# marco-conciatori-public/weed_instance_segmentation

Measured on NVIDIA B200. Metric: msda_fwd_bwd_throughput, higher is better.
Workload: dtype bf16

## Files before the change

include/msda_b200.h:

```cpp
#ifndef MSDA_B200_H_
#define MSDA_B200_H_

#include <stddef.h>
#include <stdint.h>

#ifdef __cplusplus
extern "C" {
#endif

#define MSDA_B200_ABI_VERSION 12
#define MSDA_B200_MAX_LEVELS 8

#define MSDA_B200_F32 0
#define MSDA_B200_BF16 1
#define MSDA_B200_U8 2

#define MSDA_B200_OK 0
#define MSDA_B200_ERR_INVALID 1
#define MSDA_B200_ERR_UNSUPPORTED 2
#define MSDA_B200_ERR_CUDA 3
#define MSDA_B200_ERR_WORKSPACE 4

#define MSDA_B200_FLAG_PROFILE 1u
#define MSDA_B200_FLAG_BF16_ATOMICS 2u
#define MSDA_B200_FLAG_BWD_V1 4u
#define MSDA_B200_FLAG_BWD_V2 32u
#define MSDA_B200_FLAG_STRICT_PADDING 16u

typedef struct msda_b200_desc {
  int32_t B;
  int32_t S;
  int32_t Q;
  int32_t H;
  int32_t D;
  int32_t L;
  int32_t P;
  int32_t value_dtype;
  int32_t attn_dtype;
  uint32_t flags;
  const int32_t* spatial_shapes_hw;
  const int64_t* level_start_index;
} msda_b200_desc;

int msda_b200_abi_version(void);

const char* msda_b200_last_error(void);

int msda_b200_forward(const msda_b200_desc* desc, const void* value , const float* loc ,
                      const void* attn , void* out , const int32_t* query_order ,
                      void* stream);

size_t msda_b200_backward_workspace_bytes(const msda_b200_desc* desc);

int msda_b200_backward(const msda_b200_desc* desc, const void* value , const float* loc ,
                       const void* attn , const void* grad_out , void* grad_value ,
                       float* grad_loc , void* grad_attn , void* workspace ,
                       size_t workspace_bytes, const int32_t* query_order , void* stream);

int msda_b200_forward_fused(const msda_b200_desc* desc, const void* value , const void* offsets ,
                            const void* logits , const float* ref_points , void* out ,
                            float* attn_out , const int32_t* query_order , void* stream);

int msda_b200_backward_fused(const msda_b200_desc* desc, const void* value , const void* offsets ,
                             const void* logits , const float* ref_points , const void* grad_out ,
                             void* grad_value , void* grad_offsets , void* grad_logits ,
                             void* workspace , size_t workspace_bytes,
                             const int32_t* query_order , void* stream);

int msda_b200_add_layernorm_forward(const void* x , int x_dtype, const void* residual , int residual_dtype,
                                    const float* gamma , const float* beta , float eps, float* y ,
                                    void* y_lowp , float* mean , float* rstd ,
                                    int64_t rows, int32_t channels, void* stream);

int msda_b200_add_layernorm_backward(const float* grad_y , const void* grad_y_lowp ,
                                     const void* x , int x_dtype, const void* residual , int residual_dtype,
                                     const float* gamma , const float* mean , const float* rstd ,
                                     float* grad_sum , void* grad_sum_lowp , float* grad_gamma ,
                                     float* grad_beta , int64_t rows, int32_t channels, void* stream);

int msda_b200_add_layernorm_clamp_forward(const void* x , int x_dtype, const void* residual ,
                                          int residual_dtype, const float* gamma , const float* beta ,
                                          float eps, float clamp, float* y , void* y_lowp ,
                                          float* mean , float* rstd , int64_t rows,
                                          int32_t channels, void* stream);

int msda_b200_add_layernorm_clamp_backward(const float* grad_y , const void* grad_y_lowp ,
                                           const void* x , int x_dtype, const void* residual ,
                                           int residual_dtype, const float* gamma , const float* beta ,
                                           float clamp, const float* mean , const float* rstd ,
                                           float* grad_sum , void* grad_sum_lowp ,
                                           float* grad_gamma , float* grad_beta , int64_t rows,
                                           int32_t channels, void* stream);

// ... 73 lines not shown
```

weed_instance_segmentation_b200/_cabi.py:

```python
from __future__ import annotations

import ctypes
import os

PKG = os.path.dirname(os.path.abspath(__file__))
LIB_PATH = os.path.join(PKG, "libmsda_b200.so")

ABI_VERSION = 12
MAX_LEVELS = 8
F32, BF16, U8 = 0, 1, 2
FLAG_PROFILE = 1
FLAG_BF16_ATOMICS = 2
FLAG_BWD_V1 = 4
FLAG_STRICT_PADDING = 16
FLAG_BWD_V2 = 32
PROF_FWD, PROF_BWD_ZERO, PROF_BWD_MAIN, PROF_BWD_CONVERT = 0, 1, 2, 3

EXPORTS = (
    "msda_b200_abi_version",
    "msda_b200_last_error",
    "msda_b200_forward",
    "msda_b200_backward_workspace_bytes",
    "msda_b200_backward",
    "msda_b200_forward_fused",
    "msda_b200_backward_fused",
    "msda_b200_add_layernorm_forward",
    "msda_b200_add_layernorm_backward",
    "msda_b200_add_layernorm_clamp_forward",
    "msda_b200_add_layernorm_clamp_backward",
    "msda_b200_query_value_cast_forward",
    "msda_b200_query_value_cast_backward",
    "msda_b200_relu_backward_column_sum",
    "msda_b200_linear_f32_available",
    "msda_b200_linear_f32_forward",
    "msda_b200_linear_f32_grad_input",
    "msda_b200_linear_f32_grad_weight",
    "msda_b200_column_sum",
    "msda_b200_groupnorm_to_rows_forward",
    "msda_b200_groupnorm_to_rows_backward",
    "msda_b200_point_sample_forward",
    "msda_b200_point_sample_backward",
    "msda_b200_host_pipeline_create",
    "msda_b200_host_pipeline_step",
    "msda_b200_host_pipeline_join",
    "msda_b200_host_pipeline_sync",
    "msda_b200_host_pipeline_destroy",
    "msda_b200_profile_ms",
    "msda_b200_launch_count",
)


class Desc(ctypes.Structure):

    _fields_ = [
        ("B", ctypes.c_int32), ("S", ctypes.c_int32), ("Q", ctypes.c_int32), ("H", ctypes.c_int32),
        ("D", ctypes.c_int32), ("L", ctypes.c_int32), ("P", ctypes.c_int32),
        ("value_dtype", ctypes.c_int32), ("attn_dtype", ctypes.c_int32), ("flags", ctypes.c_uint32),
        ("spatial_shapes_hw", ctypes.POINTER(ctypes.c_int32)),
        ("level_start_index", ctypes.POINTER(ctypes.c_int64)),
    ]


class MSDAError(RuntimeError):

    def __init__(self, code: int, message: str):
        super().__init__(f"msda_b200 error {code}: {message}")
        self.code = code


_lib = None


def load() -> ctypes.CDLL:
    global _lib
    if _lib is not None:
        return _lib
    if not os.path.exists(LIB_PATH):
        raise ImportError(
            f"{LIB_PATH} is missing. Build it with `python -m weed_instance_segmentation_b200.build` "
            "(needs nvcc). This package has no CPU fallback."
        )
    lib = ctypes.CDLL(LIB_PATH)
    vp = ctypes.c_void_p
    dp = ctypes.POINTER(Desc)
    lib.msda_b200_abi_version.restype = ctypes.c_int
    lib.msda_b200_abi_version.argtypes = []
    lib.msda_b200_last_error.restype = ctypes.c_char_p
    lib.msda_b200_last_error.argtypes = []
    lib.msda_b200_forward.restype = ctypes.c_int
    lib.msda_b200_forward.argtypes = [dp, vp, vp, vp, vp, vp, vp]
    lib.msda_b200_backward_workspace_bytes.restype = ctypes.c_size_t
# ... 102 lines not shown
```

weed_instance_segmentation_b200/csrc/msda_b200.cu:

```cuda
#include <cuda_bf16.h>
#include <cuda_runtime.h>

#include <atomic>
#include <cstdarg>
#include <cstdio>
#include <cstring>
#include <type_traits>

#include "msda_b200.h"

namespace {

#include "msda_common.cuh"

template <int NT, int LPP, int QPG>
struct Tile {
  static constexpr int NG = NT / LPP;
  static constexpr int TQ = NG * QPG;
  static constexpr int ROW = TQ + 1;
};

__device__ __forceinline__ void decode_block(const KParams& p, int& b, int& tile, int& h) {
  int bid = blockIdx.x;
  h = bid % p.H;
  bid /= p.H;
  tile = bid % p.num_tiles;
  b = bid / p.num_tiles;
}

template <typename AT>
__device__ __forceinline__ float2 load_pair(const void* base, long long idx);
template <>
__device__ __forceinline__ float2 load_pair<float>(const void* base, long long idx) {
  return __ldg(reinterpret_cast<const float2*>(base) + idx);
}
template <>
__device__ __forceinline__ float2 load_pair<__nv_bfloat16>(const void* base, long long idx) {
  const __nv_bfloat162 v = reinterpret_cast<const __nv_bfloat162*>(base)[idx];
  return make_float2(__low2float(v), __high2float(v));
}
template <typename AT>
__device__ __forceinline__ void store_pair(void* base, long long idx, float x, float y);
template <>
__device__ __forceinline__ void store_pair<float>(void* base, long long idx, float x, float y) {
  reinterpret_cast<float2*>(base)[idx] = make_float2(x, y);
}
template <>
__device__ __forceinline__ void store_pair<__nv_bfloat16>(void* base, long long idx, float x, float y) {
  reinterpret_cast<__nv_bfloat162*>(base)[idx] = __floats2bfloat162_rn(x, y);
}

__device__ __forceinline__ float2 implicit_reference_point(const KParams& p, int q) {
  int lq = 0;
  for (int l = 1; l < p.L; ++l)
    if (q >= p.lv[l].start) lq = l;
  const int r = q - p.lv[lq].start, W = p.lv[lq].W, H = p.lv[lq].H;
  const int y = r / W, x = r - y * W;
  return make_float2(__fdiv_rn((float)x + 0.5f, (float)W), __fdiv_rn((float)y + 0.5f, (float)H));
}

template <typename AT>
__device__ __forceinline__ float2 fused_loc(const KParams& p, long long si, long long ri, int q, const Level& lv) {
  const float2 off = load_pair<AT>(p.offsets, si);
  const float2 r = p.ref ? __ldg(reinterpret_cast<const float2*>(p.ref) + ri) : implicit_reference_point(p, q);
  return make_float2(__fadd_rn(r.x, __fdiv_rn(off.x, (float)lv.W)), __fadd_rn(r.y, __fdiv_rn(off.y, (float)lv.H)));
}

template <typename AT>
__device__ __forceinline__ void softmax_stats(const AT* lg, int LP, float& mx, float& inv) {
  mx = -INFINITY;
  for (int s = 0; s < LP; ++s) mx = fmaxf(mx, to_float<AT>(lg[s]));
  float sum = 0.f;
  for (int s = 0; s < LP; ++s) sum += expf(to_float<AT>(lg[s]) - mx);
  inv = 1.f / sum;
}

template <typename AT>
__device__ __forceinline__ void softmax_stats_x4(const AT* lg, int LP, int sub, bool valid, float& mx, float& inv) {
  mx = -INFINITY;
  if (valid)
    for (int s = sub; s < LP; s += 4) mx = fmaxf(mx, to_float<AT>(lg[s]));
  mx = fmaxf(mx, __shfl_xor_sync(0xffffffffu, mx, 1));
  mx = fmaxf(mx, __shfl_xor_sync(0xffffffffu, mx, 2));
  float sum = 0.f;
  if (valid)
    for (int s = sub; s < LP; s += 4) sum += expf(to_float<AT>(lg[s]) - mx);
  sum += __shfl_xor_sync(0xffffffffu, sum, 1);
  sum += __shfl_xor_sync(0xffffffffu, sum, 2);
  inv = valid ? 1.f / sum : 0.f;
}

template <typename AT, int NT, int HPB>
__device__ __forceinline__ void tile_softmax(const KParams& p, int b, int h0, int q0, int nq, float* s_att, bool write_out) {
  const int LP = p.LP;
  const int sub = threadIdx.x & 3;
  const int nv = nq * HPB;
  for (int vb0 = 0; vb0 < nv; vb0 += NT / 4) {
    const int v = vb0 + (threadIdx.x >> 2);
    const bool valid = v < nv;
    const int ql = v / HPB, h = h0 + v % HPB;
    const int q = valid ? (p.q_order ? p.q_order[q0 + ql] : q0 + ql) : 0;
    const long long row = (((long long)b * p.Q + q) * p.H + h) * LP;
    const AT* lg = reinterpret_cast<const AT*>(p.logits) + row;
    if (LP <= 16) {
      float e[4];
      float mx = -INFINITY;
#pragma unroll
      for (int r = 0; r < 4; ++r) {
        const int s = sub + 4 * r;
        e[r] = (valid && s < LP) ? to_float<AT>(lg[s]) : -INFINITY;
// ... 564 lines not shown
    return fail(MSDA_B200_ERR_CUDA, "forward: cannot reserve %zu bytes of shared memory", smem);
  cudaFuncSetAttribute(kern, cudaFuncAttributePreferredSharedMemoryCarveout, FUSED ? -1 : 50);
  const long long blocks = (long long)p.B * p.num_tiles * (p.H / HPB);
  if (blocks > 0x7fffffffll) return fail(MSDA_B200_ERR_UNSUPPORTED, "forward: grid too large");
  {
    ProfScope ps((d->flags & MSDA_B200_FLAG_PROFILE) != 0, MSDA_B200_PROF_FWD, st);
    kern<<<(unsigned)blocks, NT, smem, st>>>(p);
    ++g_launches;
  }
  return check_launch("msda_b200_forward (head pairs)");
}

template <typename VT, typename AT, int D, int ACC, bool FUSED>
int launch_bwd(const msda_b200_desc* d, KParams p, cudaStream_t st) {
  constexpr int LPP = D / Vec16<VT>::N;
  using T = Tile<kBwdNT, LPP, kBwdQPG>;
  fill_geometry(d, p, T::TQ);
  const size_t n = (size_t)p.LP * T::ROW;
  const size_t smem = n * (2 * sizeof(float4) + sizeof(float) + sizeof(int)) +
                      (size_t)p.LP * T::TQ * LPP * sizeof(float4) +
                      (FUSED ? 2 * (size_t)T::TQ * p.LP * sizeof(float) : 0);
  auto kern = msda_bwd_kernel<VT, AT, D, kBwdNT, kBwdQPG, ACC, FUSED>;
  if (smem > 48 * 1024 &&
      cudaFuncSetAttribute(kern, cudaFuncAttributeMaxDynamicSharedMemorySize, (int)smem) != cudaSuccess)
    return fail(MSDA_B200_ERR_CUDA, "backward: cannot reserve %zu bytes of shared memory", smem);
  const long long blocks = (long long)p.B * p.num_tiles * p.H;
  if (blocks > 0x7fffffffll) return fail(MSDA_B200_ERR_UNSUPPORTED, "backward: grid too large");
  {
    ProfScope ps((d->flags & MSDA_B200_FLAG_PROFILE) != 0, MSDA_B200_PROF_BWD_MAIN, st);
    kern<<<(unsigned)blocks, kBwdNT, smem, st>>>(p);
    ++g_launches;
  }
  return check_launch("msda_b200_backward");
}

template <typename VT, typename AT, bool FUSED>
int dispatch_fwd(const msda_b200_desc* d, const KParams& p, cudaStream_t st) {
  if constexpr (std::is_same<VT, __nv_bfloat16>::value) {
    if (d->D == 32 && d->H % 2 == 0 && !(d->flags & MSDA_B200_FLAG_STRICT_PADDING))
      return launch_fwd_pair<VT, AT, 32, FUSED>(d, p, st);
  }
  switch (d->D) {
    case 8: return launch_fwd<VT, AT, 8, FUSED>(d, p, st);
    case 128: return launch_fwd<VT, AT, 128, FUSED>(d, p, st);
    case 16: return launch_fwd<VT, AT, 16, FUSED>(d, p, st);
    case 32: return launch_fwd<VT, AT, 32, FUSED>(d, p, st);
    case 64: return launch_fwd<VT, AT, 64, FUSED>(d, p, st);
  }
  return fail(MSDA_B200_ERR_UNSUPPORTED, "head dim %d", d->D);
}

constexpr int kSortNT = 256, kSortTQ = 128, kSortCAP = 2048;

bool sorted_applicable(const msda_b200_desc* d) {
  if (d->flags & MSDA_B200_FLAG_BWD_V1) return false;
  if (d->D != 32 || d->P != 4) return false;
  if (d->value_dtype != MSDA_B200_BF16) return false;
  for (int l = 0; l < d->L; ++l)
    if (d->spatial_shapes_hw[2 * l] > 4095 || d->spatial_shapes_hw[2 * l + 1] > 4095) return false;
  return true;
}

template <typename VT, typename AT, int ACC, bool FUSED, int kNT, int kTQ, int kPL>
int launch_bwd_sorted_cfg(const msda_b200_desc* d, KParams p, cudaStream_t st) {
  constexpr int D = 32, P = 4;
  constexpr int LPP = D / Vec16<VT>::N;
  fill_geometry(d, p, kTQ);
  const size_t smem = sorted_smem_layout<kNT, kTQ, P, kSortCAP, LPP>().total;
  auto kern = msda_bwd_sorted_kernel<VT, AT, D, kNT, kTQ, P, kSortCAP, ACC, FUSED, kPL>;
  if (cudaFuncSetAttribute(kern, cudaFuncAttributeMaxDynamicSharedMemorySize, (int)smem) != cudaSuccess)
    return fail(MSDA_B200_ERR_CUDA, "backward: cannot reserve %zu bytes of shared memory", smem);
  const long long blocks = (long long)p.B * p.num_tiles * p.H;
  if (blocks > 0x7fffffffll) return fail(MSDA_B200_ERR_UNSUPPORTED, "backward: grid too large");
  {
    ProfScope ps((d->flags & MSDA_B200_FLAG_PROFILE) != 0, MSDA_B200_PROF_BWD_MAIN, st);
    kern<<<(unsigned)blocks, kNT, smem, st>>>(p);
    ++g_launches;
  }
  return check_launch("msda_b200_backward (sorted)");
}

constexpr int kMmaNT = 256, kMmaTQ = 128, kMmaGCAP = 256, kMmaRCAP = 1024;

template <typename AT, bool FUSED>
int launch_bwd_mma(const msda_b200_desc* d, KParams p, cudaStream_t st) {
  constexpr int P = 4;
  fill_geometry(d, p, kMmaTQ);
  const size_t smem = mma_smem_layout<kMmaNT, kMmaTQ, P, kMmaGCAP, kMmaRCAP, FUSED>().total;
  auto kern = msda_bwd_mma_kernel<AT, kMmaNT, kMmaTQ, P, kMmaGCAP, kMmaRCAP, FUSED>;
  if (cudaFuncSetAttribute(kern, cudaFuncAttributeMaxDynamicSharedMemorySize, (int)smem) != cudaSuccess)
    return fail(MSDA_B200_ERR_CUDA, "backward: cannot reserve %zu bytes of shared memory", smem);
  const long long blocks = (long long)p.B * p.num_tiles * p.H;
  if (blocks > 0x7fffffffll) return fail(MSDA_B200_ERR_UNSUPPORTED, "backward: grid too large");
  {
    ProfScope ps((d->flags & MSDA_B200_FLAG_PROFILE) != 0, MSDA_B200_PROF_BWD_MAIN, st);
    kern<<<(unsigned)blocks, kMmaNT, smem, st>>>(p);
    ++g_launches;
  }
  return check_launch("msda_b200_backward (group-sorted, mma)");
}

template <typename VT, typename AT, int ACC, bool FUSED>
int dispatch_bwd(const msda_b200_desc* d, const KParams& p, cudaStream_t st) {
  if constexpr (std::is_same<VT, __nv_bfloat16>::value) {
    if (sorted_applicable(d)) {
      if constexpr (ACC == 0) {
        if (!(d->flags & MSDA_B200_FLAG_BWD_V2)) return launch_bwd_mma<AT, FUSED>(d, p, st);
      }
      return launch_bwd_sorted_cfg<VT, AT, ACC, FUSED, kSortNT, kSortTQ, 4>(d, p, st);
    }
  }
  switch (d->D) {
    case 8: return launch_bwd<VT, AT, 8, ACC, FUSED>(d, p, st);
    case 128: return launch_bwd<VT, AT, 128, ACC, FUSED>(d, p, st);
    case 16: return launch_bwd<VT, AT, 16, ACC, FUSED>(d, p, st);
    case 32: return launch_bwd<VT, AT, 32, ACC, FUSED>(d, p, st);
    case 64: return launch_bwd<VT, AT, 64, ACC, FUSED>(d, p, st);
  }
  return fail(MSDA_B200_ERR_UNSUPPORTED, "head dim %d", d->D);
}

template <bool FUSED>
int run_forward(const msda_b200_desc* desc, const KParams& p, cudaStream_t st) {
  const bool vbf = desc->value_dtype == MSDA_B200_BF16, abf = desc->attn_dtype == MSDA_B200_BF16;
  if (!vbf) return dispatch_fwd<float, float, FUSED>(desc, p, st);
  if (abf) return dispatch_fwd<__nv_bfloat16, __nv_bfloat16, FUSED>(desc, p, st);
  return dispatch_fwd<__nv_bfloat16, float, FUSED>(desc, p, st);
}

template <bool FUSED>
int run_backward(const msda_b200_desc* desc, KParams p, void* grad_value, void* workspace, size_t workspace_bytes,
                 bool have_tensors, cudaStream_t st) {
  const bool prof = (desc->flags & MSDA_B200_FLAG_PROFILE) != 0;
  const bool vbf = desc->value_dtype == MSDA_B200_BF16, abf = desc->attn_dtype == MSDA_B200_BF16;
  const bool bf16_atomics = vbf && (desc->flags & MSDA_B200_FLAG_BF16_ATOMICS);
  const size_t nvalue = (size_t)desc->B * desc->S * desc->H * desc->D;
  const size_t need = msda_b200_backward_workspace_bytes(desc);
  if (nvalue && !grad_value) return fail(MSDA_B200_ERR_INVALID, "backward: grad_value is NULL");
  if (need && nvalue && (!workspace || workspace_bytes < need))
    return fail(MSDA_B200_ERR_WORKSPACE, "backward: workspace of %zu bytes required, got %zu", need, workspace_bytes);
  if (nvalue && need && (reinterpret_cast<uintptr_t>(workspace) & 15))
    return fail(MSDA_B200_ERR_INVALID, "backward: workspace must be 16-byte aligned");

  void* acc = need ? workspace : grad_value;
  if (nvalue) {
    ProfScope ps(prof, MSDA_B200_PROF_BWD_ZERO, st);
    const size_t acc_bytes = need ? need : nvalue * dtype_size(desc->value_dtype);
    if (cudaMemsetAsync(acc, 0, acc_bytes, st) != cudaSuccess) return check_launch("backward: memset");
  }
  if ((long long)desc->B * desc->Q != 0) {
    if (!have_tensors) return fail(MSDA_B200_ERR_INVALID, "backward: NULL tensor pointer");
    p.grad_value_acc = acc;
    int rc;
    if (!vbf) rc = dispatch_bwd<float, float, 0, FUSED>(desc, p, st);
    else if (bf16_atomics) rc = abf ? dispatch_bwd<__nv_bfloat16, __nv_bfloat16, 1, FUSED>(desc, p, st)
                                    : dispatch_bwd<__nv_bfloat16, float, 1, FUSED>(desc, p, st);
    else rc = abf ? dispatch_bwd<__nv_bfloat16, __nv_bfloat16, 0, FUSED>(desc, p, st)
                  : dispatch_bwd<__nv_bfloat16, float, 0, FUSED>(desc, p, st);
    if (rc) return rc;
  }
  if (need && nvalue) {
    ProfScope ps(prof, MSDA_B200_PROF_BWD_CONVERT, st);
    const long long n8 = (long long)(nvalue / 8);
    const int blocks = (int)((n8 + 255) / 256 < 148 * 16 ? (n8 + 255) / 256 : 148 * 16);
    msda_cvt_f32_bf16_kernel<<<blocks, 256, 0, st>>>(reinterpret_cast<const float4*>(workspace),
                                                     reinterpret_cast<uint4*>(grad_value), n8);
    ++g_launches;
    if (int rc = check_launch("backward: convert")) return rc;
  }
  return MSDA_B200_OK;
}

}

extern "C" {

int msda_b200_internal_fail(int code, const char* msg) { return fail(code, "%s", msg); }
int msda_b200_internal_validate(const msda_b200_desc* desc) { return validate(desc); }
void msda_b200_internal_count_launch(void) { ++g_launches; }

int msda_b200_abi_version(void) { return MSDA_B200_ABI_VERSION; }

const char* msda_b200_last_error(void) { return g_err; }

int msda_b200_forward(const msda_b200_desc* desc, const void* value, const float* loc, const void* attn, void* out,
                      const int32_t* query_order, void* stream) {
  g_err[0] = 0;
  if (int rc = validate(desc)) return rc;
  if ((long long)desc->B * desc->Q == 0) return MSDA_B200_OK;
  if (!value || !loc || !attn || !out) return fail(MSDA_B200_ERR_INVALID, "forward: NULL tensor pointer");
  KParams p;
  memset(&p, 0, sizeof(p));
  p.value = value; p.loc = loc; p.attn = attn; p.out = out; p.q_order = query_order;
  return run_forward<false>(desc, p, reinterpret_cast<cudaStream_t>(stream));
}

int msda_b200_forward_fused(const msda_b200_desc* desc, const void* value, const void* offsets, const void* logits,
                            const float* ref_points, void* out, float* attn_out, const int32_t* query_order,
                            void* stream) {
  g_err[0] = 0;
  if (int rc = validate(desc)) return rc;
  if ((long long)desc->B * desc->Q == 0) return MSDA_B200_OK;
  if (!value || !offsets || !logits || !out) return fail(MSDA_B200_ERR_INVALID, "forward_fused: NULL tensor pointer");
  if (!ref_points && desc->Q != desc->S)
    return fail(MSDA_B200_ERR_INVALID, "forward_fused: implicit reference points (ref_points = NULL) need Q == S");
  KParams p;
  memset(&p, 0, sizeof(p));
  p.value = value; p.offsets = offsets; p.logits = logits; p.ref = ref_points; p.out = out; p.attn_out = attn_out;
  p.q_order = query_order;
  return run_forward<true>(desc, p, reinterpret_cast<cudaStream_t>(stream));
}

size_t msda_b200_backward_workspace_bytes(const msda_b200_desc* desc) {
  if (!desc) return 0;
  if (desc->value_dtype == MSDA_B200_BF16 && !(desc->flags & MSDA_B200_FLAG_BF16_ATOMICS))
    return (size_t)desc->B * desc->S * desc->H * desc->D * sizeof(float);
  return 0;
}

int msda_b200_backward(const msda_b200_desc* desc, const void* value, const float* loc, const void* attn,
                       const void* grad_out, void* grad_value, float* grad_loc, void* grad_attn, void* workspace,
                       size_t workspace_bytes, const int32_t* query_order, void* stream) {
  g_err[0] = 0;
  if (int rc = validate(desc)) return rc;
  KParams p;
  memset(&p, 0, sizeof(p));
  p.value = value; p.loc = loc; p.attn = attn; p.grad_out = grad_out;
  p.grad_loc = grad_loc; p.grad_attn = grad_attn; p.q_order = query_order;
  const bool have = value && loc && attn && grad_out && grad_loc && grad_attn;
  return run_backward<false>(desc, p, grad_value, workspace, workspace_bytes, have, reinterpret_cast<cudaStream_t>(stream));
}

int msda_b200_backward_fused(const msda_b200_desc* desc, const void* value, const void* offsets, const void* logits,
                             const float* ref_points, const void* grad_out, void* grad_value, void* grad_offsets,
                             void* grad_logits, void* workspace, size_t workspace_bytes, const int32_t* query_order,
                             void* stream) {
  g_err[0] = 0;
  if (int rc = validate(desc)) return rc;
  KParams p;
  memset(&p, 0, sizeof(p));
  p.value = value; p.offsets = offsets; p.logits = logits; p.ref = ref_points; p.grad_out = grad_out;
  p.grad_offsets = grad_offsets; p.grad_logits = grad_logits; p.q_order = query_order;
  if (!ref_points && desc->Q != desc->S)
    return fail(MSDA_B200_ERR_INVALID, "backward_fused: implicit reference points (ref_points = NULL) need Q == S");
  const bool have = value && offsets && logits && grad_out && grad_offsets && grad_logits;
  return run_backward<true>(desc, p, grad_value, workspace, workspace_bytes, have, reinterpret_cast<cudaStream_t>(stream));
}

int msda_b200_profile_ms(int which, float* ms) {
  if (which < 0 || which >= MSDA_B200_PROF_COUNT || !ms) return fail(MSDA_B200_ERR_INVALID, "profile_ms: bad argument");
  if (g_prof.device < 0 || !g_prof.valid[which]) return fail(MSDA_B200_ERR_INVALID, "profile_ms: nothing recorded");
  const cudaError_t e = cudaEventElapsedTime(ms, g_prof.ev[which][0], g_prof.ev[which][1]);
  if (e != cudaSuccess) return fail(MSDA_B200_ERR_CUDA, "profile_ms: %s", cudaGetErrorString(e));
  return MSDA_B200_OK;
}

int64_t msda_b200_launch_count(int reset) {
  return reset ? g_launches.exchange(0) : g_launches.load();
}

}
```

weed_instance_segmentation_b200/csrc/msda_bwd_mma.cuh:

```cuda

__device__ __forceinline__ void ldsm_x4(unsigned (&r)[4], unsigned addr) {
  asm("ldmatrix.sync.aligned.m8n8.x4.shared.b16 {%0, %1, %2, %3}, [%4];"
      : "=r"(r[0]), "=r"(r[1]), "=r"(r[2]), "=r"(r[3]) : "r"(addr));
}
__device__ __forceinline__ void ldsm_x4_trans(unsigned (&r)[4], unsigned addr) {
  asm("ldmatrix.sync.aligned.m8n8.x4.trans.shared.b16 {%0, %1, %2, %3}, [%4];"
      : "=r"(r[0]), "=r"(r[1]), "=r"(r[2]), "=r"(r[3]) : "r"(addr));
}
__device__ __forceinline__ void ldsm_x2_trans(unsigned (&r)[2], unsigned addr) {
  asm("ldmatrix.sync.aligned.m8n8.x2.trans.shared.b16 {%0, %1}, [%2];" : "=r"(r[0]), "=r"(r[1]) : "r"(addr));
}
__device__ __forceinline__ unsigned movm_trans(unsigned x) {
  unsigned y;
  asm("movmatrix.sync.aligned.m8n8.trans.b16 %0, %1;" : "=r"(y) : "r"(x));
  return y;
}
__device__ __forceinline__ void mma_bf16(float (&d)[4], unsigned a0, unsigned a1, unsigned a2, unsigned a3, unsigned b0,
                                         unsigned b1) {
  asm("mma.sync.aligned.m16n8k16.row.col.f32.bf16.bf16.f32 {%0, %1, %2, %3}, {%4, %5, %6, %7}, {%8, %9}, "
      "{%0, %1, %2, %3};"
      : "+f"(d[0]), "+f"(d[1]), "+f"(d[2]), "+f"(d[3]) : "r"(a0), "r"(a1), "r"(a2), "r"(a3), "r"(b0), "r"(b1));
}

__device__ __forceinline__ int go_swizzle(int row) { return ((row >> 1) & 1) | ((row >> 3) & 2); }

#ifndef MSDA_MMA_MOVM
#define MSDA_MMA_MOVM 1
#endif

struct MmaSmem {
  size_t w, go, wrow, dot, a, xy, cnt, item, id, fb, misc, stat, total;
};

constexpr int kMmaItemRows = 64;

template <int NT, int TQ, int P, int GCAP, int RCAP, bool FUSED>
__host__ __device__ inline MmaSmem mma_smem_layout() {
  constexpr int NS = TQ * P;
  MmaSmem s;
  size_t o = 0;
  s.w = o;    o += sizeof(float4) * NS;
  s.go = o;   o += 64 * (TQ + 1);
  s.wrow = o; o += 16 * RCAP;
  s.dot = o;  o += sizeof(float4) * NS;
  s.a = o;    o += sizeof(float) * NS;
  s.xy = o;   o += sizeof(int) * NS;
  s.cnt = o;  o += sizeof(int) * GCAP;
  s.item = o; o += sizeof(uint2) * (GCAP + RCAP / kMmaItemRows + 8);
  s.id = o;   o += sizeof(unsigned) * RCAP;
  s.fb = o;   o += sizeof(unsigned short) * NS * 4;
  o = (o + 15) & ~size_t(15);
  s.misc = o; o += sizeof(int) * 64;
  s.stat = o;
  s.total = o;
  return s;
}

enum { MI_NITEMS = 9 };

template <typename AT, int NT, int TQ, int P, int GCAP, int RCAP, bool FUSED>
__global__ void __launch_bounds__(NT, 4) msda_bwd_mma_kernel(const __grid_constant__ KParams p) {
  using VT = __nv_bfloat16;
  constexpr int LPP = 4;
  constexpr int G = NT / LPP;
  constexpr int NS = TQ * P;
  constexpr int LP2 = Log2P<P>::v;
  constexpr int NW = NT / 32;
  static_assert(GCAP == NT, "the scan gives every thread one group counter");
  static_assert(NS % NT == 0, "every thread owns NS/NT samples per level");
  static_assert(NS <= 512, "row code: 9 bits of sample index");
  static_assert(RCAP < 2048 && RCAP % 16 == 0, "row index is 11 bits in the item word");
  extern __shared__ __align__(16) unsigned char smem_raw[];
  const MmaSmem lay = mma_smem_layout<NT, TQ, P, GCAP, RCAP, FUSED>();
  float4* s_w = reinterpret_cast<float4*>(smem_raw + lay.w);
  unsigned* s_go32 = reinterpret_cast<unsigned*>(smem_raw + lay.go);
  uint4* s_wrow = reinterpret_cast<uint4*>(smem_raw + lay.wrow);
  float* s_dot = reinterpret_cast<float*>(smem_raw + lay.dot);
  float* s_a = reinterpret_cast<float*>(smem_raw + lay.a);
  int* s_xy = reinterpret_cast<int*>(smem_raw + lay.xy);
  int* s_cnt = reinterpret_cast<int*>(smem_raw + lay.cnt);
  uint2* s_item = reinterpret_cast<uint2*>(smem_raw + lay.item);
  unsigned* s_id = reinterpret_cast<unsigned*>(smem_raw + lay.id);
  unsigned short* s_fb = reinterpret_cast<unsigned short*>(smem_raw + lay.fb);
  int* const s_misc2 = reinterpret_cast<int*>(smem_raw + lay.misc);

  int b, tile, h;
  decode_block(p, b, tile, h);
  const int q0 = tile * TQ;
  const int nq = min(TQ, p.Q - q0);
  const int tid = threadIdx.x, lane = tid & 31, warp = tid >> 5;
  const int g = tid / LPP, c = tid % LPP;
  const unsigned gmask = ((1u << LPP) - 1u) << ((lane / LPP) * LPP);
  const long long acc_base = (long long)b * p.batch_stride16;
  const uint4* const vrow = reinterpret_cast<const uint4*>(p.value) + acc_base;
  float* const acc_f = reinterpret_cast<float*>(p.grad_value_acc) + acc_base * 8;
  const unsigned go_sa = (unsigned)__cvta_generic_to_shared(s_go32);
  const unsigned wrow_sa = (unsigned)__cvta_generic_to_shared(s_wrow);

  constexpr int SPT = NS / NT;
  float2 pre_loc[SPT];
  float pre_a[SPT];
  float2 f_ref[SPT];
#pragma unroll
  for (int r = 0; r < SPT; ++r) {
    f_ref[r] = make_float2(0.f, 0.f);
    const int ql = (r * NT + tid) >> LP2;
    if (FUSED && !p.ref && ql < nq) f_ref[r] = implicit_reference_point(p, p.q_order ? p.q_order[q0 + ql] : q0 + ql);
  }
  auto fetch_level = [&](int l) {
#pragma unroll
    for (int r = 0; r < SPT; ++r) {
      const int si = r * NT + tid;
      const int ql = si >> LP2, pt = si & (P - 1);
      pre_loc[r] = make_float2(0.f, 0.f);
      pre_a[r] = 0.f;
      if (l < p.L && ql < nq) {
        const int q = p.q_order ? p.q_order[q0 + ql] : q0 + ql;
        const long long gi = (((long long)b * p.Q + q) * p.H + h) * p.LP + l * P + pt;
        if (FUSED) {
          const float2 off = load_pair<AT>(p.offsets, gi);
          const float2 rp = p.ref ? __ldg(reinterpret_cast<const float2*>(p.ref) + ((long long)b * p.Q + q) * p.L + l)
                                  : f_ref[r];
          pre_loc[r] = make_float2(__fadd_rn(rp.x, __fdiv_rn(off.x, (float)p.lv[l].W)),
                                   __fadd_rn(rp.y, __fdiv_rn(off.y, (float)p.lv[l].H)));
          pre_a[r] = to_float<AT>(reinterpret_cast<const AT*>(p.logits)[gi]);
        } else {
          pre_loc[r] = __ldg(reinterpret_cast<const float2*>(p.loc) + gi);
          pre_a[r] = to_float<AT>(reinterpret_cast<const AT*>(p.attn)[gi]);
        }
      }
    }
  };
  fetch_level(0);

  for (int i = tid; i < TQ * LPP; i += NT) {
    const int ql = i >> 2, cc = i & 3;
    uint4 v = make_uint4(0u, 0u, 0u, 0u);
    if (ql < nq) {
      const int q = p.q_order ? p.q_order[q0 + ql] : q0 + ql;
      v = ldg16(reinterpret_cast<const uint4*>(p.grad_out) + (((long long)b * p.Q + q) * p.H + h) * LPP + cc);
    }
    const int sw = go_swizzle(ql);
    unsigned* row = s_go32 + ql * 16 + cc;
    row[(0 ^ sw) << 2] = __byte_perm(v.x, v.z, 0x5410);
    row[(1 ^ sw) << 2] = __byte_perm(v.x, v.z, 0x7632);
    row[(2 ^ sw) << 2] = __byte_perm(v.y, v.w, 0x5410);
    row[(3 ^ sw) << 2] = __byte_perm(v.y, v.w, 0x7632);
  }
  if (tid < 16) s_go32[TQ * 16 + tid] = 0u;

  static_assert(!FUSED || P == 4, "fused prologue: four lanes per (query, head) row");
  float f_lse[SPT], f_dsum[SPT];
#pragma unroll
  for (int r = 0; r < SPT; ++r) { f_lse[r] = 0.f; f_dsum[r] = 0.f; }
  if (FUSED) {
#pragma unroll
    for (int r = 0; r < SPT; ++r) {
      const int ql = (r * NT + tid) >> LP2;
      const bool valid = ql < nq;
      const int q = valid ? (p.q_order ? p.q_order[q0 + ql] : q0 + ql) : 0;
      float mx, inv;
      softmax_stats_x4<AT>(reinterpret_cast<const AT*>(p.logits) + (((long long)b * p.Q + q) * p.H + h) * p.LP, p.LP,
                           tid & 3, valid, mx, inv);
      f_lse[r] = valid ? mx - logf(inv) : 0.f;
    }
  }

  auto init_misc = [&](int* m) {
    int init = 0;
    if (tid == MI_MINX || tid == MI_MINY) init = 0x7fffffff;
// ... 96 lines not shown
              if (((cn & 1) ? cx1 : cx0) && ((cn & 2) ? cy1 : cy0))
                s_fb[atomicAdd(&s_misc[MI_FBN], 1)] = (unsigned short)(si * 4 + cn);
          }
        }
        code[r][k] = cd;
      }
    }
    __syncthreads();

    {
      const int cnt = s_cnt[tid];
      const int v = cnt | (((cnt + kMmaItemRows - 1) / kMmaItemRows) << 16);
      int incl = v;
#pragma unroll
      for (int off = 1; off < 32; off <<= 1) {
        const int t = __shfl_up_sync(0xffffffffu, incl, off);
        if (lane >= off) incl += t;
      }
      if (lane == 31) s_misc[MI_WSUM + warp] = incl;
      __syncthreads();
      int base = 0;
#pragma unroll
      for (int w2 = 0; w2 < NW; ++w2)
        if (w2 < warp) base += s_misc[MI_WSUM + w2];
      const int excl = base + incl - v;
      const int row_start = excl & 0xffff, item_start = excl >> 16;
      s_cnt[tid] = row_start;
      if (tid == NT - 1) {
        s_misc[MI_TOTAL] = (excl + v) & 0xffff;
        s_misc[MI_NITEMS] = (excl + v) >> 16;
      }
      if (cnt > 0) {
        const int gyl = tid / gw, gxl = tid - gyl * gw;
        const int px0 = (gx_lo + gxl) << 2, py0 = (gy_lo + gyl) << 1;
        const unsigned xbits = (1u << min(lv.W - px0, 4)) - 1u;
        const unsigned mask = xbits | (py0 + 1 < lv.H ? xbits << 4 : 0u);
        const unsigned pixoff = (unsigned)((py0 * lv.W + px0) * (p.H * LPP));
        for (int j = 0; j * kMmaItemRows < cnt; ++j) {
          const int rb = row_start + j * kMmaItemRows;
          const int n = rb < RCAP ? min(min(kMmaItemRows, cnt - j * kMmaItemRows), RCAP - rb) : 0;
          s_item[item_start + j] = make_uint2((unsigned)(n ? rb : 0) | ((unsigned)n << 11) | (mask << 18), pixoff);
        }
      }
    }
    __syncthreads();

#pragma unroll
    for (int r = 0; r < SPT; ++r) {
      const int si = r * NT + tid;
      const int xy = s_xy[si];
      const int x = xy & 0xfff, y = (xy >> 12) & 0xfff;
      const float4 w = s_w[si];
      const float a = s_a[si];
#pragma unroll
      for (int k = 0; k < 4; ++k) {
        const int cd = code[r][k];
        if (cd >= 0) {
          const int ci = k & 1, cj = k >> 1;
          const int slot = atomicAdd(&s_cnt[cd], 1);
          if (slot < RCAP) {
            const int bx = ci ? -1 : (x & 3), by = cj ? -1 : (y & 1);
            const int ql = si >> LP2;
            s_id[slot] = (unsigned)(ql * 64 + (go_swizzle(ql) << 4)) | ((unsigned)(si | ((bx + 1) << 9) | ((by + 1) << 12)) << 14);
            const float y0w = by == 0 ? a * w.z : (by == -1 ? a * w.w : 0.f);
            const float y1w = by == 1 ? a * w.z : (by == 0 ? a * w.w : 0.f);
            const unsigned p0 = Vec16<VT>::pack2(y0w * w.x, y0w * w.y), p1 = Vec16<VT>::pack2(y1w * w.x, y1w * w.y);
            const unsigned long long r0 = bx >= 0 ? ((unsigned long long)p0 << (16 * bx)) : (unsigned long long)(p0 >> 16);
            const unsigned long long r1 = bx >= 0 ? ((unsigned long long)p1 << (16 * bx)) : (unsigned long long)(p1 >> 16);
            s_wrow[slot] = make_uint4((unsigned)r0, (unsigned)(r0 >> 32), (unsigned)r1, (unsigned)(r1 >> 32));
          } else {
            const int gcode = xy >> 24;
            const bool ax0 = (gcode & 3) != 1, ax1 = ((gcode >> 2) & 3) != 1;
            const bool ay0 = ((gcode >> 4) & 3) != 1, ay1 = ((gcode >> 6) & 3) != 1;
            const bool xsplit = (x & 3) == 3, ysplit = (y & 1) == 1;
            const bool cx0 = (ci == 0) && ax0, cx1 = ax1 && (ci == 0 ? !xsplit : xsplit);
            const bool cy0 = (cj == 0) && ay0, cy1 = ay1 && (cj == 0 ? !ysplit : ysplit);
#pragma unroll
            for (int cn = 0; cn < 4; ++cn)
              if (((cn & 1) ? cx1 : cx0) && ((cn & 2) ? cy1 : cy0))
                s_fb[atomicAdd(&s_misc[MI_FBN], 1)] = (unsigned short)(si * 4 + cn);
          }
        }
      }
    }
    __syncthreads();
    s_cnt[tid] = 0;

    {
      const int g8 = lane >> 2, t4 = lane & 3;
      const int n_items = s_misc[MI_NITEMS];
      const int pix16 = p.H * LPP;
      const uint4* const v_lane = vrow + (lv.start * p.H + h) * LPP + ((g8 >> 2) * lv.W + (g8 & 3)) * pix16 + t4;
      float* const acc_lane = acc_f + (long long)((lv.start * p.H + h) * LPP + ((t4 >> 1) * lv.W + 2 * (t4 & 1)) * pix16) * 8 + 4 * g8;
      const int kx = 2 * (t4 & 1) + 1, ky = (t4 >> 1) + 1;
      const unsigned vbit = 1u << (18 + g8), fbit = 1u << (18 + 2 * t4);
      const unsigned lsel = ((unsigned)lane >> 4) << 4;
      auto load_v = [&](uint2 item) -> uint4 {
        if (item.x & vbit) return ldg16(v_lane + (int)item.y);
        return make_uint4(0u, 0u, 0u, 0u);
      };
      int it = warp;
      uint2 item = it < n_items ? s_item[it] : make_uint2(0u, 0u);
      uint4 vv = load_v(item);
      while (it < n_items) {
        const int it_n = it + NW;
        const uint2 item_n = it_n < n_items ? s_item[it_n] : make_uint2(0u, 0u);
        const uint4 vv_n = load_v(item_n);
        const int n = (int)((item.x >> 11) & 127u);
        if (n != 0) {
          const int rbeg = (int)(item.x & 0x7ffu), rend = rbeg + n;
          const unsigned bv00 = __byte_perm(vv.x, vv.z, 0x5410);
          const unsigned bv01 = __byte_perm(vv.x, vv.z, 0x7632);
          const unsigned bv10 = __byte_perm(vv.y, vv.w, 0x5410);
          const unsigned bv11 = __byte_perm(vv.y, vv.w, 0x7632);
          float acc0[4] = {0.f, 0.f, 0.f, 0.f}, acc1[4] = {0.f, 0.f, 0.f, 0.f};
          const unsigned kNoRow = 0x0fffc000u | (unsigned)(TQ * 64);
          int r0 = rbeg;
          unsigned code_l = r0 + (lane & 15) < rend ? s_id[r0 + (lane & 15)] : kNoRow;
          while (true) {
            const int rn = r0 + 16;
            const unsigned code_ln = rn + (lane & 15) < rend ? s_id[rn + (lane & 15)] : kNoRow;
            const int idx = r0 + (lane & 15);
            const unsigned ga = go_sa + ((code_l & 0x3fffu) ^ lsel);
            unsigned a[4], a2[4], tA[4], tB[4], bw[2];
            ldsm_x4(a, ga);
            ldsm_x4(a2, ga ^ 32u);
#if MSDA_MMA_MOVM
#pragma unroll
            for (int j = 0; j < 4; ++j) { tA[j] = movm_trans(a[j]); tB[j] = movm_trans(a2[j]); }
#else
            ldsm_x4_trans(tA, ga);
            ldsm_x4_trans(tB, ga ^ 32u);
#endif
            ldsm_x2_trans(bw, idx < rend ? wrow_sa + idx * 16 : go_sa + TQ * 64);
            float d[4] = {0.f, 0.f, 0.f, 0.f};
            mma_bf16(d, a[0], a[1], a[2], a[3], bv00, bv01);
            mma_bf16(d, a2[0], a2[1], a2[2], a2[3], bv10, bv11);
            mma_bf16(acc0, tA[0], tA[2], tA[1], tA[3], bw[0], bw[1]);
            mma_bf16(acc1, tB[0], tB[2], tB[1], tB[3], bw[0], bw[1]);
#pragma unroll
            for (int e = 0; e < 2; ++e) {
              const unsigned code = __shfl_sync(0xffffffffu, code_l, g8 + 8 * e);
              const int cxa = kx - (int)((code >> 23) & 7u), cy = ky - (int)((code >> 26) & 3u);
              float* dst = s_dot + ((code >> 14) & 511u) * 4 + cy * 2 + cxa;
              if ((unsigned)cy < 2u && (unsigned)cxa < 2u) dst[0] = d[2 * e];
              if ((unsigned)cy < 2u && (unsigned)(cxa + 1) < 2u) dst[1] = d[2 * e + 1];
            }
            if (rn >= rend) break;
            r0 = rn; code_l = code_ln;
          }
          float* const dst = acc_lane + (long long)(int)item.y * 8;
#pragma unroll
          for (int s = 0; s < 2; ++s) {
            const float v0 = acc0[s], v1 = acc0[2 + s], v2 = acc1[s], v3 = acc1[2 + s];
            const unsigned nz = (__float_as_uint(v0) | __float_as_uint(v1) | __float_as_uint(v2) | __float_as_uint(v3)) << 1;
            if ((item.x & (fbit << s)) && nz != 0u) red_add_f32x4(dst + s * pix16 * 8, v0, v1, v2, v3);
          }
        }
        it = it_n; item = item_n; vv = vv_n;
      }
    }

    fetch_level(l + 1);

    {
      const int nfb = s_misc[MI_FBN];
// ... 6 lines not shown
        const int x = (xy & 0xfff) + (cn & 1), y = ((xy >> 12) & 0xfff) + ((cn >> 1) & 1);
        const long long off = (long long)((lv.start + y * lv.W + x) * p.H + h) * LPP;
        float vf[8], gf[8];
        Vec16<VT>::unpack(ldg16(vrow + off + c), vf);
        {
          const int ql = si >> LP2, sw = go_swizzle(ql);
          const unsigned* row = s_go32 + ql * 16 + c;
#pragma unroll
          for (int j = 0; j < 4; ++j) {
            const unsigned u = row[(j ^ sw) << 2];
            gf[j] = __uint_as_float(u << 16);
            gf[j + 4] = __uint_as_float(u & 0xffff0000u);
          }
        }
        float d = 0.f;
#pragma unroll
        for (int j = 0; j < 8; ++j) d = fmaf(gf[j], vf[j], d);
#pragma unroll
        for (int o = 1; o < LPP; o <<= 1) d += __shfl_xor_sync(gmask, d, o);
        if (c == 0) s_dot[id] = d;
        if (wgt != 0.f) {
          float* dst = acc_f + (off + c) * 8;
          red_add_f32x4(dst, wgt * gf[0], wgt * gf[1], wgt * gf[2], wgt * gf[3]);
          red_add_f32x4(dst + 4, wgt * gf[4], wgt * gf[5], wgt * gf[6], wgt * gf[7]);
        }
      }
    }
    __syncthreads();

#pragma unroll
    for (int r = 0; r < SPT; ++r) {
      const int si = r * NT + tid;
      const int ql = si >> LP2, pt = si & (P - 1);
      const bool valid = ql < nq;
      const int q = valid ? (p.q_order ? p.q_order[q0 + ql] : q0 + ql) : 0;
      const long long gi = (((long long)b * p.Q + q) * p.H + h) * p.LP + l * P + pt;
      float4 d = *reinterpret_cast<const float4*>(&s_dot[si * 4]);
      const float4 w = s_w[si];
      const int gcode = s_xy[si] >> 24;
      const float a = s_a[si];
      const float gl = gdec(gcode, 0), gr = gdec(gcode, 1), gt = gdec(gcode, 2), gb = gdec(gcode, 3);
      d.x = (gl != 0.f && gt != 0.f) ? d.x : 0.f;
      d.y = (gr != 0.f && gt != 0.f) ? d.y : 0.f;
      d.z = (gl != 0.f && gb != 0.f) ? d.z : 0.f;
      d.w = (gr != 0.f && gb != 0.f) ? d.w : 0.f;
      const float top_s = w.x * d.x + w.y * d.y, bot_s = w.x * d.z + w.y * d.w;
      const float top_g = gl * d.x + gr * d.y, bot_g = gl * d.z + gr * d.w;
      const float g_attn = w.z * top_s + w.w * bot_s;
      const float g_px = w.z * top_g + w.w * bot_g, g_py = gt * top_s + gb * bot_s;
      if (!FUSED) {
        if (valid) {
          reinterpret_cast<AT*>(p.grad_attn)[gi] = from_float<AT>(g_attn);
          reinterpret_cast<float2*>(p.grad_loc)[gi] = make_float2((float)lv.W * a * g_px, (float)lv.H * a * g_py);
        }
      } else {
        if (valid) {
          store_pair<AT>(p.grad_offsets, gi, a * g_px, a * g_py);
          reinterpret_cast<AT*>(p.grad_logits)[gi] = from_float<AT>(g_attn);
        }
        float t = valid ? a * g_attn : 0.f;
#pragma unroll
        for (int o = 1; o < P; o <<= 1) t += __shfl_xor_sync(0xffffffffu, t, o);
        f_dsum[r] += t;
      }
    }
  }

  if (FUSED) {
#pragma unroll
    for (int r = 0; r < SPT; ++r) {
      const int ql = (r * NT + tid) >> LP2, pt = tid & (P - 1);
      if (ql < nq) {
        const int q = p.q_order ? p.q_order[q0 + ql] : q0 + ql;
        const long long row = (((long long)b * p.Q + q) * p.H + h) * p.LP;
        for (int l = 0; l < p.L; ++l) {
          const long long gi = row + l * P + pt;
          const float a = expf(to_float<AT>(reinterpret_cast<const AT*>(p.logits)[gi]) - f_lse[r]);
          const float ga = to_float<AT>(reinterpret_cast<const AT*>(p.grad_logits)[gi]);
          reinterpret_cast<AT*>(p.grad_logits)[gi] = from_float<AT>(a * (ga - f_dsum[r]));
        }
      }
    }
  }
}
```

weed_instance_segmentation_b200/csrc/msda_common.cuh:

```cuda
#pragma once

constexpr int kMaxL = MSDA_B200_MAX_LEVELS;

struct Level {
  int H, W;
  int start;
  int dx16;
  int dy16;
};

struct KParams {
  const void* value;
  const float* loc;
  const void* attn;
  void* out;
  const void* grad_out;
  void* grad_value_acc;
  float* grad_loc;
  void* grad_attn;
  const int* q_order;
  const void* offsets;
  const void* logits;
  const float* ref;
  float* attn_out;
  void* grad_offsets;
  void* grad_logits;
  int B, S, Q, H, L, P, LP;
  int num_tiles;
  long long batch_stride16;
  Level lv[kMaxL];
};

struct Axis {
  float s0, s1;
  float g0, g1;
  int base;
  bool ok;
};

__device__ __forceinline__ Axis axis_setup(float coord, int n) {
  Axis a;
  const float g = __fadd_rn(__fmul_rn(2.f, coord), -1.f);
  const float pix = __fmul_rn(__fadd_rn(__fmul_rn(__fadd_rn(g, 1.f), (float)n), -1.f), 0.5f);
  a.ok = (pix > -2.f) && (pix < (float)(n + 1));
  const float fl = floorf(pix);
  const int i0 = __float2int_rd(pix);
  const float l = pix - fl;
  const bool v0 = (i0 >= 0) && (i0 < n);
  const bool v1 = (i0 + 1 >= 0) && (i0 + 1 < n);
  const float w0 = v0 ? 1.f - l : 0.f, w1 = v1 ? l : 0.f;
  const float d0 = v0 ? -1.f : 0.f, d1 = v1 ? 1.f : 0.f;
  const int ib = min(max(i0, 0), max(n - 2, 0));
  const int shift = i0 - ib;
  a.base = ib;
  a.s0 = (shift == 0) ? w0 : ((shift == -1) ? w1 : 0.f);
  a.g0 = (shift == 0) ? d0 : ((shift == -1) ? d1 : 0.f);
  a.s1 = (shift == 0) ? w1 : ((shift == 1) ? w0 : 0.f);
  a.g1 = (shift == 0) ? d1 : ((shift == 1) ? d0 : 0.f);
  if (!a.ok) a.s0 = a.s1 = a.g0 = a.g1 = 0.f;
  return a;
}

template <typename T>
__device__ __forceinline__ float to_float(T v);
template <>
__device__ __forceinline__ float to_float<float>(float v) { return v; }
template <>
__device__ __forceinline__ float to_float<__nv_bfloat16>(__nv_bfloat16 v) { return __bfloat162float(v); }

template <typename T>
__device__ __forceinline__ T from_float(float v);
template <>
__device__ __forceinline__ float from_float<float>(float v) { return v; }
template <>
__device__ __forceinline__ __nv_bfloat16 from_float<__nv_bfloat16>(float v) { return __float2bfloat16_rn(v); }

template <typename T>
struct Vec16;
template <>
struct Vec16<float> {
  static constexpr int N = 4;
  static __device__ __forceinline__ void unpack(const uint4& v, float (&f)[4]) {
    f[0] = __uint_as_float(v.x); f[1] = __uint_as_float(v.y);
    f[2] = __uint_as_float(v.z); f[3] = __uint_as_float(v.w);
  }
  static __device__ __forceinline__ uint4 pack(const float (&f)[4]) {
    return make_uint4(__float_as_uint(f[0]), __float_as_uint(f[1]), __float_as_uint(f[2]), __float_as_uint(f[3]));
  }
};
template <>
struct Vec16<__nv_bfloat16> {
  static constexpr int N = 8;
  static __device__ __forceinline__ void unpack(const uint4& v, float (&f)[8]) {
    f[0] = __uint_as_float(v.x << 16); f[1] = __uint_as_float(v.x & 0xffff0000u);
    f[2] = __uint_as_float(v.y << 16); f[3] = __uint_as_float(v.y & 0xffff0000u);
    f[4] = __uint_as_float(v.z << 16); f[5] = __uint_as_float(v.z & 0xffff0000u);
    f[6] = __uint_as_float(v.w << 16); f[7] = __uint_as_float(v.w & 0xffff0000u);
  }
  static __device__ __forceinline__ unsigned pack2(float lo, float hi) {
    __nv_bfloat162 h = __floats2bfloat162_rn(lo, hi);
    return *reinterpret_cast<unsigned*>(&h);
  }
  static __device__ __forceinline__ uint4 pack(const float (&f)[8]) {
    return make_uint4(pack2(f[0], f[1]), pack2(f[2], f[3]), pack2(f[4], f[5]), pack2(f[6], f[7]));
  }
};

__device__ __forceinline__ uint4 ldg16(const uint4* p) { return __ldg(p); }

// ... 30 lines not shown
```

Baseline: 6610.

## Fuse grad_value zeroing and bf16 conversion into MMA backward kernel via ticket sync

Blocks of the MMA backward kernel now take dynamic tickets. Each block zeroes a slice of the next batch's fp32 accumulator while working on the current batch, and converts an earlier batch's accumulator to bf16 once all of that batch's blocks have signalled done. Extra tail blocks convert the last batches. This replaces the full-workspace memset with a memset of one batch plus the sync counters, and drops the separate convert kernel launch, with the aim of overlapping that memory traffic with compute. In exchange it adds spin-waits on global counters between blocks, which risks stalls, and it depends on ticket order matching forward progress.

```diff
diff --git a/include/msda_b200.h b/include/msda_b200.h
--- a/include/msda_b200.h
+++ b/include/msda_b200.h
@@ -8,7 +8,7 @@
 extern "C" {
 #endif
 
-#define MSDA_B200_ABI_VERSION 12
+#define MSDA_B200_ABI_VERSION 13
 #define MSDA_B200_MAX_LEVELS 8
 
 #define MSDA_B200_F32 0
diff --git a/weed_instance_segmentation_b200/_cabi.py b/weed_instance_segmentation_b200/_cabi.py
--- a/weed_instance_segmentation_b200/_cabi.py
+++ b/weed_instance_segmentation_b200/_cabi.py
@@ -6,7 +6,7 @@
 PKG = os.path.dirname(os.path.abspath(__file__))
 LIB_PATH = os.path.join(PKG, "libmsda_b200.so")
 
-ABI_VERSION = 12
+ABI_VERSION = 13
 MAX_LEVELS = 8
 F32, BF16, U8 = 0, 1, 2
 FLAG_PROFILE = 1
diff --git a/weed_instance_segmentation_b200/csrc/msda_b200.cu b/weed_instance_segmentation_b200/csrc/msda_b200.cu
--- a/weed_instance_segmentation_b200/csrc/msda_b200.cu
+++ b/weed_instance_segmentation_b200/csrc/msda_b200.cu
@@ -1,6 +1,7 @@
 #include <cuda_bf16.h>
 #include <cuda_runtime.h>
 
+#include <algorithm>
 #include <atomic>
 #include <cstdarg>
 #include <cstdio>
@@ -20,12 +21,14 @@
   static constexpr int ROW = TQ + 1;
 };
 
-__device__ __forceinline__ void decode_block(const KParams& p, int& b, int& tile, int& h) {
-  int bid = blockIdx.x;
+__device__ __forceinline__ void decode_index(const KParams& p, int bid, int& b, int& tile, int& h) {
   h = bid % p.H;
   bid /= p.H;
   tile = bid % p.num_tiles;
   b = bid / p.num_tiles;
+}
+__device__ __forceinline__ void decode_block(const KParams& p, int& b, int& tile, int& h) {
+  decode_index(p, blockIdx.x, b, tile, h);
 }
 
 template <typename AT>
@@ -756,6 +759,12 @@
 
 constexpr int kMmaNT = 256, kMmaTQ = 128, kMmaGCAP = 256, kMmaRCAP = 1024;
 
+bool mma_applicable(const msda_b200_desc* d) {
+  return d->value_dtype == MSDA_B200_BF16 && !(d->flags & (MSDA_B200_FLAG_BF16_ATOMICS | MSDA_B200_FLAG_BWD_V2)) &&
+         d->spatial_shapes_hw && sorted_applicable(d);
+}
+size_t mma_sync_bytes(const msda_b200_desc* d) { return ((size_t)(1 + 2 * d->B) * sizeof(unsigned) + 15) & ~size_t(15); }
+
 template <typename AT, bool FUSED>
 int launch_bwd_mma(const msda_b200_desc* d, KParams p, cudaStream_t st) {
   constexpr int P = 4;
@@ -764,7 +773,8 @@
   auto kern = msda_bwd_mma_kernel<AT, kMmaNT, kMmaTQ, P, kMmaGCAP, kMmaRCAP, FUSED>;
   if (cudaFuncSetAttribute(kern, cudaFuncAttributeMaxDynamicSharedMemorySize, (int)smem) != cudaSuccess)
     return fail(MSDA_B200_ERR_CUDA, "backward: cannot reserve %zu bytes of shared memory", smem);
-  const long long blocks = (long long)p.B * p.num_tiles * p.H;
+  const long long nbi = (long long)p.num_tiles * p.H;
+  const long long blocks = p.B * nbi + std::min(p.B, kMmaConvertLag) * ((nbi + kMmaTailChunks - 1) / kMmaTailChunks);
   if (blocks > 0x7fffffffll) return fail(MSDA_B200_ERR_UNSUPPORTED, "backward: grid too large");
   {
     ProfScope ps((d->flags & MSDA_B200_FLAG_PROFILE) != 0, MSDA_B200_PROF_BWD_MAIN, st);
@@ -816,15 +826,22 @@
   if (nvalue && need && (reinterpret_cast<uintptr_t>(workspace) & 15))
     return fail(MSDA_B200_ERR_INVALID, "backward: workspace must be 16-byte aligned");
 
-  void* acc = need ? workspace : grad_value;
+  const bool launched = (long long)desc->B * desc->Q != 0;
+  const size_t sync_bytes = need && mma_applicable(desc) ? mma_sync_bytes(desc) : 0;
+  const bool duties = sync_bytes && launched;
+  void* acc = need ? static_cast<char*>(workspace) + sync_bytes : grad_value;
   if (nvalue) {
     ProfScope ps(prof, MSDA_B200_PROF_BWD_ZERO, st);
-    const size_t acc_bytes = need ? need : nvalue * dtype_size(desc->value_dtype);
-    if (cudaMemsetAsync(acc, 0, acc_bytes, st) != cudaSuccess) return check_launch("backward: memset");
-  }
-  if ((long long)desc->B * desc->Q != 0) {
+    const size_t acc_bytes = need ? need - sync_bytes : nvalue * dtype_size(desc->value_dtype);
+    const cudaError_t e = duties ? cudaMemsetAsync(workspace, 0, sync_bytes + acc_bytes / desc->B, st)
+                                 : cudaMemsetAsync(acc, 0, acc_bytes, st);
+    if (e != cudaSuccess) return check_launch("backward: memset");
+  }
+  if (launched) {
     if (!have_tensors) return fail(MSDA_B200_ERR_INVALID, "backward: NULL tensor pointer");
     p.grad_value_acc = acc;
+    p.bwd_sync = duties ? static_cast<unsigned*>(workspace) : nullptr;
+    p.grad_value_out = grad_value;
     int rc;
     if (!vbf) rc = dispatch_bwd<float, float, 0, FUSED>(desc, p, st);
     else if (bf16_atomics) rc = abf ? dispatch_bwd<__nv_bfloat16, __nv_bfloat16, 1, FUSED>(desc, p, st)
@@ -835,12 +852,14 @@
   }
   if (need && nvalue) {
     ProfScope ps(prof, MSDA_B200_PROF_BWD_CONVERT, st);
-    const long long n8 = (long long)(nvalue / 8);
-    const int blocks = (int)((n8 + 255) / 256 < 148 * 16 ? (n8 + 255) / 256 : 148 * 16);
-    msda_cvt_f32_bf16_kernel<<<blocks, 256, 0, st>>>(reinterpret_cast<const float4*>(workspace),
-                                                     reinterpret_cast<uint4*>(grad_value), n8);
-    ++g_launches;
-    if (int rc = check_launch("backward: convert")) return rc;
+    if (!duties) {
+      const long long n8 = (long long)(nvalue / 8);
+      const int blocks = (int)((n8 + 255) / 256 < 148 * 16 ? (n8 + 255) / 256 : 148 * 16);
+      msda_cvt_f32_bf16_kernel<<<blocks, 256, 0, st>>>(reinterpret_cast<const float4*>(acc),
+                                                       reinterpret_cast<uint4*>(grad_value), n8);
+      ++g_launches;
+      if (int rc = check_launch("backward: convert")) return rc;
+    }
   }
   return MSDA_B200_OK;
 }
@@ -887,8 +906,10 @@
 
 size_t msda_b200_backward_workspace_bytes(const msda_b200_desc* desc) {
   if (!desc) return 0;
-  if (desc->value_dtype == MSDA_B200_BF16 && !(desc->flags & MSDA_B200_FLAG_BF16_ATOMICS))
-    return (size_t)desc->B * desc->S * desc->H * desc->D * sizeof(float);
+  if (desc->value_dtype == MSDA_B200_BF16 && !(desc->flags & MSDA_B200_FLAG_BF16_ATOMICS)) {
+    const size_t acc = (size_t)desc->B * desc->S * desc->H * desc->D * sizeof(float);
+    return acc && mma_applicable(desc) ? mma_sync_bytes(desc) + acc : acc;
+  }
   return 0;
 }
 
diff --git a/weed_instance_segmentation_b200/csrc/msda_bwd_mma.cuh b/weed_instance_segmentation_b200/csrc/msda_bwd_mma.cuh
--- a/weed_instance_segmentation_b200/csrc/msda_bwd_mma.cuh
+++ b/weed_instance_segmentation_b200/csrc/msda_bwd_mma.cuh
@@ -56,7 +56,51 @@
   return s;
 }
 
-enum { MI_NITEMS = 9 };
+enum { MI_NITEMS = 9, MI_TICKET = 24 };
+
+constexpr int kMmaConvertLag = 2;
+constexpr int kMmaTailChunks = 4;
+
+__device__ __forceinline__ unsigned ld_relaxed_gpu(const unsigned* a) {
+  unsigned v;
+  asm volatile("ld.relaxed.gpu.global.u32 %0, [%1];" : "=r"(v) : "l"(a) : "memory");
+  return v;
+}
+__device__ __forceinline__ unsigned ld_acquire_gpu(const unsigned* a) {
+  unsigned v;
+  asm volatile("ld.acquire.gpu.global.u32 %0, [%1];" : "=r"(v) : "l"(a) : "memory");
+  return v;
+}
+__device__ __forceinline__ void count_release(unsigned* a) {
+  asm volatile("red.release.gpu.global.add.u32 [%0], 1;" ::"l"(a) : "memory");
+}
+__device__ __forceinline__ void count_wait(const unsigned* a, unsigned n) {
+  while (ld_relaxed_gpu(a) < n) __nanosleep(200);
+  (void)ld_acquire_gpu(a);
+}
+
+template <int NT>
+__device__ __forceinline__ void acc_zero_units(float* acc, long long u0, long long u1) {
+  float4* const d = reinterpret_cast<float4*>(acc);
+  const float4 z = make_float4(0.f, 0.f, 0.f, 0.f);
+  for (long long u = u0 + threadIdx.x; u < u1; u += NT) { d[2 * u] = z; d[2 * u + 1] = z; }
+}
+template <int NT>
+__device__ __forceinline__ void acc_convert_units(const float* acc, void* out, long long u0, long long u1) {
+  const float4* const s = reinterpret_cast<const float4*>(acc);
+  uint4* const d = reinterpret_cast<uint4*>(out);
+  for (long long u = u0 + threadIdx.x; u < u1; u += 2 * NT) {
+    const bool two = u + NT < u1;
+    const float4 a = __ldcg(s + 2 * u), b2 = __ldcg(s + 2 * u + 1);
+    float4 c = make_float4(0.f, 0.f, 0.f, 0.f), e = c;
+    if (two) { c = __ldcg(s + 2 * (u + NT)); e = __ldcg(s + 2 * (u + NT) + 1); }
+    const float f[8] = {a.x, a.y, a.z, a.w, b2.x, b2.y, b2.z, b2.w};
+    __stcs(d + u, Vec16<__nv_bfloat16>::pack(f));
+    const float f2[8] = {c.x, c.y, c.z, c.w, e.x, e.y, e.z, e.w};
+    if (two) __stcs(d + u + NT, Vec16<__nv_bfloat16>::pack(f2));
+  }
+}
+
 
 template <typename AT, int NT, int TQ, int P, int GCAP, int RCAP, bool FUSED>
 __global__ void __launch_bounds__(NT, 4) msda_bwd_mma_kernel(const __grid_constant__ KParams p) {
@@ -84,8 +128,32 @@
   unsigned short* s_fb = reinterpret_cast<unsigned short*>(smem_raw + lay.fb);
   int* const s_misc2 = reinterpret_cast<int*>(smem_raw + lay.misc);
 
+  unsigned* const zero_ready = p.bwd_sync + 1;
+  unsigned* const done = p.bwd_sync + 1 + p.B;
+  const int nbi = p.num_tiles * p.H;
+  const long long n8 = p.batch_stride16, chunk = (n8 + nbi - 1) / nbi;
+  if (threadIdx.x == 0) s_misc2[MI_TICKET] = (int)atomicAdd(p.bwd_sync, 1u);
+  __syncthreads();
+  const int ticket = s_misc2[MI_TICKET];
+  if (ticket >= p.B * nbi) {
+    const int u = ticket - p.B * nbi, tpi = (nbi + kMmaTailChunks - 1) / kMmaTailChunks;
+    const int c = max(p.B - kMmaConvertLag, 0) + u / tpi;
+    const long long j0 = (long long)(u % tpi) * kMmaTailChunks;
+    if (threadIdx.x == 0) count_wait(done + c, nbi);
+    __syncthreads();
+    acc_convert_units<NT>(reinterpret_cast<const float*>(p.grad_value_acc) + c * n8 * 8,
+                          reinterpret_cast<uint4*>(p.grad_value_out) + c * n8, j0 * chunk,
+                          min((j0 + kMmaTailChunks) * chunk, n8));
+    return;
+  }
   int b, tile, h;
-  decode_block(p, b, tile, h);
+  decode_index(p, ticket, b, tile, h);
+  if (b + 1 < p.B) {
+    const long long j = ticket - b * nbi;
+    acc_zero_units<NT>(reinterpret_cast<float*>(p.grad_value_acc) + (b + 1) * n8 * 8, j * chunk,
+                       min((j + 1) * chunk, n8));
+  }
+
   const int q0 = tile * TQ;
   const int nq = min(TQ, p.Q - q0);
   const int tid = threadIdx.x, lane = tid & 31, warp = tid >> 5;
@@ -348,6 +416,10 @@
           }
         }
       }
+    }
+    if (l == 0 && tid == 0) {
+      if (b + 1 < p.B) count_release(zero_ready + b + 1);
+      if (b > 0) count_wait(zero_ready + b, nbi);
     }
     __syncthreads();
     s_cnt[tid] = 0;
@@ -520,4 +592,14 @@
       }
     }
   }
-}
+
+  if (tid == 0) count_release(done + b);
+  if (b >= kMmaConvertLag) {
+    const int c = b - kMmaConvertLag;
+    const long long j = s_misc2[MI_TICKET] - b * nbi;
+    if (tid == 0) count_wait(done + c, nbi);
+    __syncthreads();
+    acc_convert_units<NT>(reinterpret_cast<const float*>(p.grad_value_acc) + c * n8 * 8,
+                          reinterpret_cast<uint4*>(p.grad_value_out) + c * n8, j * chunk, min((j + 1) * chunk, n8));
+  }
+}
diff --git a/weed_instance_segmentation_b200/csrc/msda_common.cuh b/weed_instance_segmentation_b200/csrc/msda_common.cuh
--- a/weed_instance_segmentation_b200/csrc/msda_common.cuh
+++ b/weed_instance_segmentation_b200/csrc/msda_common.cuh
@@ -25,6 +25,8 @@
   float* attn_out;
   void* grad_offsets;
   void* grad_logits;
+  unsigned* bwd_sync;
+  void* grad_value_out;
   int B, S, Q, H, L, P, LP;
   int num_tiles;
   long long batch_stride16;
```

New measurement: 6369 (median of 6 runs). 0.964x the previous value.
